# Lymphatus/caesium-clt

Measured on NVIDIA H100. Metric: megapixels/sec JPEG q=80 4K re-encode, higher is better.
Workload: dtype i32

## Files before the change

caesium-clt_b200/csrc/jpeg_gpuenc.cu:

```cuda
#include <cuda_runtime.h>
#include <cub/device/device_scan.cuh>
#include <cuda_pipeline.h>
#include <algorithm>
#include <chrono>
#include <cstring>
#include "jpeg_gpuenc.h"
#include "stream_wait.h"
#include "launch_timer.h"

namespace b200 {

using namespace ge;

__global__ void k_ge_groups(const Scan *__restrict__ scans, const uint32_t *__restrict__ meta, const int *__restrict__ evkey,
                            const int *__restrict__ prev, const uint32_t *__restrict__ tsum, uint32_t *__restrict__ gcount, uint32_t *__restrict__ hist)
{
    __shared__ uint32_t eob[16];
    const Scan s = scans[blockIdx.y];
    if (s.mode != MODE_AC_FIRST && s.mode != MODE_AC_REFINE) return;
    if ((int)(blockIdx.x * blockDim.x) > s.nblocks) return;
    if (threadIdx.x < 16) eob[threadIdx.x] = 0;
    __syncthreads();
    const int b = blockIdx.x * blockDim.x + threadIdx.x;
    if (b <= s.nblocks && (b == s.nblocks || meta_event(meta[s.unit_base + b]))) {
        int pg;
        if (b < s.nblocks) pg = prev[s.unit_base + b];
        else { const long long last = s.unit_base + s.nblocks - 1; pg = max(prev[last], evkey[last]); }
        const int pl = pg >= s.unit_base ? (int)(pg - s.unit_base) : -1;
        assign_groups(meta + s.unit_base, tsum + s.unit_base, s.nblocks, pl, b, gcount + s.unit_base,
                      [&](uint32_t c) { atomicAdd(&eob[eob_symbol(c) >> 4], 1u); });
    }
    __syncthreads();
    if (threadIdx.x < 16 && eob[threadIdx.x]) atomicAdd(&hist[((size_t)s.tab_base + 2 + s.tbl[0]) * 256 + (threadIdx.x << 4)], eob[threadIdx.x]);
}

__global__ void k_ge_tables(const uint32_t *__restrict__ hist, Table *__restrict__ tabs, DhtOut *__restrict__ dht, unsigned long long *__restrict__ tbits)
{
    __shared__ long long freq[257];
    __shared__ int codesize[257], others[257];
    __shared__ uint8_t bits[33];
    const int t = blockIdx.x, lane = threadIdx.x;
    const uint32_t *f = hist + (size_t)t * 256;
    for (int i = lane; i < 257; i += 32) { freq[i] = i < 256 ? (long long)f[i] : 1; codesize[i] = 0; others[i] = -1; }
    if (lane == 0) for (int i = 0; i < 33; i++) bits[i] = 0;
    __syncwarp();
    auto warp_argmin = [&](int exclude) {
        unsigned long long v = 1000000000ULL; int c = -1;
        for (int i = lane; i < 257; i += 32) { const unsigned long long fi = (unsigned long long)freq[i]; if (fi && fi <= v && i != exclude) { v = fi; c = i; } }
        const unsigned hi = (unsigned)(v >> 32), lo = (unsigned)v;
        const unsigned mhi = __reduce_min_sync(0xFFFFFFFFu, hi);
        const unsigned mlo = __reduce_min_sync(0xFFFFFFFFu, hi == mhi ? lo : 0xFFFFFFFFu);
        return __reduce_max_sync(0xFFFFFFFFu, (hi == mhi && lo == mlo) ? c : -1);
    };
    for (;;) {
        const int c1 = warp_argmin(-1);
        const int c2 = c1 < 0 ? -1 : warp_argmin(c1);
        if (c2 < 0) break;
        if (lane == 0) {
            int a = c1, b = c2;
            freq[a] += freq[b]; freq[b] = 0;
            codesize[a]++; while (others[a] >= 0) { a = others[a]; codesize[a]++; }
            others[a] = b;
            codesize[b]++; while (others[b] >= 0) { b = others[b]; codesize[b]++; }
        }
        __syncwarp();
    }
    if (lane == 0) {
        Table &T = tabs[t];
        for (int i = 0; i <= 256; i++) if (codesize[i]) bits[codesize[i] > 32 ? 32 : codesize[i]]++;
        for (int i = 32; i > 16; i--) while (bits[i] > 0) {
            int j = i - 2; while (bits[j] == 0) j--;
            bits[i] -= 2; bits[i - 1]++; bits[j + 1] += 2; bits[j]--;
        }
        int i = 16; while (i > 0 && bits[i] == 0) i--;
        if (i > 0) bits[i]--;
        int start[34];
        for (int l = 0; l < 34; l++) start[l] = 0;
        for (int s = 0; s <= 255; s++) if (codesize[s]) start[min(codesize[s], 32) + 1]++;
        for (int l = 1; l < 34; l++) start[l] += start[l - 1];
        const int p = start[33];
        for (int s = 0; s <= 255; s++) if (codesize[s]) T.vals[start[min(codesize[s], 32)]++] = (uint8_t)s;
        T.nvals = p;
        for (int k = 0; k < 17; k++) T.bits[k] = bits[k];
        for (int s = 0; s < 256; s++) T.code_len[s] = 0;
        uint32_t code = 0; int k = 0;
        for (int l = 1; l <= 16; l++) { for (int n = 0; n < bits[l]; n++, k++) T.code_len[T.vals[k]] = (code++ << 8) | (uint32_t)l; code <<= 1; }
        DhtOut &D = dht[t];
        D.nvals = p;
        for (int k2 = 0; k2 < 17; k2++) D.bits[k2] = bits[k2];
        for (int k2 = 0; k2 < p; k2++) D.vals[k2] = T.vals[k2];
    }
    __syncwarp();
    const int kind = (t & 3) >> 1;
    unsigned long long nb = 0;
    for (int i = lane; i < 256; i += 32) if (f[i]) nb += (unsigned long long)f[i] * ((tabs[t].code_len[i] & 0xFFu) + (unsigned)sym_extra_bits(kind, i));
    for (int d = 16; d; d >>= 1) nb += __shfl_xor_sync(0xFFFFFFFFu, nb, d);
    if (lane == 0) tbits[t] = nb;
}

__global__ void k_ge_scanout(const Scan *__restrict__ scans, int nscans, const unsigned long long *__restrict__ tbits, const uint32_t *__restrict__ corr,
                             uint32_t *__restrict__ total, ScanOut *__restrict__ so, uint32_t words_cap, uint32_t groups_cap, uint32_t *__restrict__ flags)
{
    const int lane = threadIdx.x;
    uint32_t wbase = 0, gbase = 0, abase = 0;
    for (int c0 = 0; c0 < nscans; c0 += 32) {
        const int i = c0 + lane;
        uint32_t tb = 0, na = 0;
        if (i < nscans) {
            tb = (uint32_t)(tbits[4 * i] + tbits[4 * i + 1] + tbits[4 * i + 2] + tbits[4 * i + 3] + corr[i]);
            na = scans[i].nruns ? (tb + 31) / 32 + scans[i].nruns : 0;
        }
        const uint32_t nbytes = (tb + 7) / 8, ng = (nbytes + 15) / 16, nw = i < nscans ? (tb + 31) / 32 + 1 : 0;
        uint32_t wi = nw, gi = i < nscans ? ng : 0, ai = na;
        for (int d = 1; d < 32; d <<= 1) {
            const uint32_t a = __shfl_up_sync(0xFFFFFFFFu, wi, d), b = __shfl_up_sync(0xFFFFFFFFu, gi, d), c = __shfl_up_sync(0xFFFFFFFFu, ai, d);
            if (lane >= d) { wi += a; gi += b; ai += c; }
        }
        if (i < nscans) {
            total[i] = tb;
            ScanOut o; o.total_bits = tb; o.nbytes = nbytes; o.ngroups = ng; o.group_base = gbase + gi - ng; o.word_base = wbase + wi - nw; o.arena_base = abase + ai - na;
            so[i] = o;
        }
        wbase += __shfl_sync(0xFFFFFFFFu, wi, 31); gbase += __shfl_sync(0xFFFFFFFFu, gi, 31); abase += __shfl_sync(0xFFFFFFFFu, ai, 31);
    }
    __syncwarp();
    const bool ovf = wbase > words_cap || gbase > groups_cap;
    if (lane == 0) { flags[0] = ovf ? 1u : 0u; flags[1] = wbase; flags[2] = gbase; flags[3] = 0; flags[4] = 0; }
    if (ovf) for (int i = lane; i < nscans; i += 32) { so[i].total_bits = 0; so[i].nbytes = 0; so[i].ngroups = 0; so[i].group_base = 0; so[i].word_base = 0; so[i].arena_base = 0; }
}

__global__ void k_ge_zero(const Scan *__restrict__ scans, const ScanOut *__restrict__ so, uint32_t *__restrict__ words, uint32_t *__restrict__ arena)
{
    const ScanOut o = so[blockIdx.y];
    if (!o.total_bits) return;
    const uint32_t n = (o.total_bits + 31) / 32 + 1, nruns = (uint32_t)scans[blockIdx.y].nruns, na = nruns ? n - 1 + nruns : 0;
    uint32_t *w = words + o.word_base, *a = arena + o.arena_base;
    for (uint32_t i = blockIdx.x * blockDim.x + threadIdx.x; i < max(n, na); i += gridDim.x * blockDim.x) {
        if (i < n) w[i] = 0;
        if (i < na) a[i] = 0;
    }
}

constexpr int TILE_PITCH = 72;
typedef int16_t Tile[ENC_THREADS][TILE_PITCH];

__device__ __forceinline__ void stage_tile(Tile &tile, const BlockComp &bc, int i0, int nblk)
{
    const uint4 *src = reinterpret_cast<const uint4 *>(bc.coef + bc.comp_off + (long long)i0 * 64);
    const int n = min(ENC_THREADS, nblk - i0) * 8;
#pragma unroll
    for (int k = 0; k < 8; k++) { const int q = threadIdx.x + k * ENC_THREADS; if (q < n) __pipeline_memcpy_async(&tile[q >> 3][(q & 7) * 8], src + q, 16); }
    __pipeline_commit();
}
__device__ __forceinline__ void wait_tile()
{
    __pipeline_wait_prior(0);
    __syncthreads();
}

__device__ __forceinline__ void stage_visits(EncVisit *vis, const BlockComp &bc)
{
    if ((int)threadIdx.x < bc.nscan) vis[threadIdx.x] = bc.visit[threadIdx.x];
}
__device__ __forceinline__ BlockRef ref_of(const EncVisit &v, const BlockComp &bc, const Tile &tile, int i0, int row, int col)
{
    BlockRef r;
    r.blk = tile[threadIdx.x]; r.prev = nullptr; r.slot = 0;
    if (v.mode == MODE_SEQ || v.mode == MODE_DC_FIRST) {
        const int p = enc_dc_prev(bc, v.ns, row, col);
        if (p >= i0 && p < i0 + ENC_THREADS) r.prev = tile[p - i0];
        else if (p >= 0) r.prev = bc.coef + bc.comp_off + (long long)p * 64;
    }
    return r;
}

template <class T>
__device__ __forceinline__ KindTabs<T> kind_tabs(T *tab, const EncVisit &v) { return KindTabs<T>{tab + ENC_DC_ENTRY, tab + v.ac_entry}; }

__device__ __forceinline__ Masks3 load_masks(const Masks3 *__restrict__ masks, const BlockComp &bc, int i)
{
    const unsigned long long *q = reinterpret_cast<const unsigned long long *>(masks + bc.mask_base + i);
    Masks3 M;
    M.m[0] = __ldg(q); M.m[1] = __ldg(q + 1); M.m[2] = __ldg(q + 2);
    return M;
}

struct SmemHist {
    KindTabs<uint32_t> h;
    __device__ void sym(int kind, int, int symbol, int, unsigned) { atomicAdd((kind ? h.ac : h.dc) + symbol, 1u); }
    __device__ void raw64(int, unsigned long long) {}
};
__global__ void __launch_bounds__(ENC_THREADS) k_geb_classify(const BlockComp *__restrict__ comps, uint32_t *__restrict__ meta, int *__restrict__ evkey,
                                                              uint32_t *__restrict__ tail, Masks3 *__restrict__ masks, uint32_t *__restrict__ hist, uint32_t *__restrict__ corr)
{
    __shared__ __align__(16) Tile tile;
    __shared__ uint32_t h[ENC_TAB_ENTRIES];
    __shared__ EncVisit vis[ENC_MAX_VISITS];
    __shared__ uint32_t vcorr[ENC_MAX_VISITS];
    const BlockComp &bc = comps[blockIdx.y];
    const int nblk = bc.bw * bc.bh, i0 = blockIdx.x * ENC_THREADS, i = i0 + threadIdx.x;
    if (i0 >= nblk) return;
    stage_tile(tile, bc, i0, nblk);
    for (int k = threadIdx.x; k < ENC_TAB_ENTRIES; k += ENC_THREADS) h[k] = 0;
    if (threadIdx.x < ENC_MAX_VISITS) vcorr[threadIdx.x] = 0;
    stage_visits(vis, bc);
    wait_tile();
    if (i < nblk) {
        const int row = i / bc.bw, col = i - row * bc.bw;
        const Masks3 M = make_masks3(tile[threadIdx.x]);
        masks[bc.mask_base + i] = M;
        for (int j = 0; j < bc.nscan; j++) {
            const EncVisit &v = vis[j];
            const int u = enc_unit_of(bc, v.ns, row, col);
            if (u < 0) continue;
            const uint32_t m = classify_m(v, M);
            const int g = v.unit_base + u;
            meta[g] = m; evkey[g] = meta_event(m) ? g : -1; tail[g] = (uint32_t)meta_tail(m);
            SmemHist sk{kind_tabs(h, v)};
            gen_block_m(v, v.tbl, ref_of(v, bc, tile, i0, row, col), M, 0, sk);
            const int nc = corr_bits_m(v, M);
            if (nc) atomicAdd(&vcorr[j], (uint32_t)nc);
        }
    }
    __syncthreads();
    if ((int)threadIdx.x < bc.nscan && vcorr[threadIdx.x]) atomicAdd(&corr[vis[threadIdx.x].scan], vcorr[threadIdx.x]);
    for (int k = threadIdx.x; k < ENC_TAB_ENTRIES; k += ENC_THREADS) {
        int symbol; const int t = enc_entry_table(bc, k, symbol);
        if (h[k]) atomicAdd(&hist[(size_t)t * 256 + symbol], h[k]);
    }
}

__global__ void __launch_bounds__(ENC_THREADS) k_geb_len(const BlockComp *__restrict__ comps, const uint32_t *__restrict__ gcount, const Table *__restrict__ tabs,
                                                         uint32_t *__restrict__ bitlen, const Masks3 *__restrict__ masks)
{
    __shared__ __align__(16) Tile tile;
    __shared__ uint8_t tl[ENC_TAB_ENTRIES];
    __shared__ EncVisit vis[ENC_MAX_VISITS];
    const BlockComp &bc = comps[blockIdx.y];
    const int nblk = bc.bw * bc.bh, i0 = blockIdx.x * ENC_THREADS, i = i0 + threadIdx.x;
    if (i0 >= nblk) return;
    stage_tile(tile, bc, i0, nblk);
    const Masks3 M = load_masks(masks, bc, min(i, nblk - 1));
    stage_visits(vis, bc);
    for (int k = threadIdx.x; k < ENC_TAB_ENTRIES; k += ENC_THREADS) {
        int symbol; const int t = enc_entry_table(bc, k, symbol);
        if (t >= 0) tl[k] = (uint8_t)tabs[t].code_len[symbol];
    }
    wait_tile();
    if (i >= nblk) return;
    const int row = i / bc.bw, col = i - row * bc.bw;
    for (int j = 0; j < bc.nscan; j++) {
        const EncVisit &v = vis[j];
        if (v.ns == 1) continue;
        const int u = enc_unit_of(bc, v.ns, row, col);
        if (u < 0) continue;
        LenSinkT<KindTabs<const uint8_t>> sk{kind_tabs<const uint8_t>(tl, v)};
        gen_block_m(v, v.tbl, ref_of(v, bc, tile, i0, row, col), M, gcount[v.unit_base + u], sk);
        bitlen[v.lu_base + u] = (uint32_t)sk.bits;
    }
}
constexpr int LEN_DC_THREADS = 256;
__global__ void __launch_bounds__(LEN_DC_THREADS) k_geb_len_dc(const BlockComp *__restrict__ comps, const Table *__restrict__ tabs, uint32_t *__restrict__ bitlen)
{
    const BlockComp &bc = comps[blockIdx.y];
    const int nblk = bc.bw * bc.bh, i = blockIdx.x * LEN_DC_THREADS + threadIdx.x;
    if (i >= nblk) return;
    const int row = i / bc.bw, col = i - row * bc.bw;
    const int16_t *cb = bc.coef + bc.comp_off;
    const Masks3 none{};
    for (int j = 0; j < bc.nscan; j++) {
        const EncVisit v = bc.visit[j];
        if (v.ns == 1) continue;
        const int p = enc_dc_prev(bc, v.ns, row, col);
        const BlockRef r{cb + (long long)i * 64, p >= 0 ? cb + (long long)p * 64 : nullptr, 0};
        LenSinkT<KindTabs<const uint32_t>> sk{KindTabs<const uint32_t>{tabs[bc.tab[ENC_AC_SLOTS]].code_len, nullptr}};
        gen_block_m(v, v.tbl, r, none, 0, sk);
        bitlen[v.lu_base + enc_unit_of(bc, v.ns, row, col)] = (uint32_t)sk.bits;
    }
}

__device__ __forceinline__ uint32_t cta_exclusive_sum(uint32_t x, uint32_t *wsum , uint32_t &total)
{
    const int lane = threadIdx.x & 31, w = threadIdx.x >> 5;
    uint32_t inc = x;
    for (int d = 1; d < 32; d <<= 1) { const uint32_t y = __shfl_up_sync(0xFFFFFFFFu, inc, d); if (lane >= d) inc += y; }
    if (lane == 31) wsum[w] = inc;
    __syncthreads();
    uint32_t base = 0, tot = 0;
#pragma unroll
    for (int k = 0; k < ENC_THREADS / 32; k++) { const uint32_t sk = wsum[k]; if (k < w) base += sk; tot += sk; }
    total = tot;
    return base + inc - x;
}

constexpr int ENC_SLOT_WORDS = 8;
__global__ void __launch_bounds__(ENC_THREADS) k_geb_emit(const BlockComp *__restrict__ comps, const uint32_t *__restrict__ gcount, const Table *__restrict__ tabs,
                                                          const uint32_t *__restrict__ bitoff, uint32_t *__restrict__ words, const Masks3 *__restrict__ masks, const ScanOut *__restrict__ so,
                                                          const uint32_t *__restrict__ flags, uint32_t *__restrict__ arena, uint32_t *__restrict__ cursor,
                                                          uint32_t *__restrict__ runlen, uint32_t *__restrict__ runpos)
{
    __shared__ __align__(16) Tile tile;
    __shared__ uint32_t tc[ENC_TAB_ENTRIES];
    __shared__ EncVisit vis[ENC_MAX_VISITS];
    __shared__ uint32_t vword[ENC_MAX_VISITS], vbit0[ENC_MAX_VISITS];
    __shared__ uint32_t slot[ENC_SLOT_WORDS][ENC_THREADS];
    __shared__ uint32_t wsum[ENC_THREADS / 32], run_word;
    if (flags[0]) return;
    const BlockComp &bc = comps[blockIdx.y];
    const int nblk = bc.bw * bc.bh, i0 = blockIdx.x * ENC_THREADS, i = i0 + threadIdx.x;
    if (i0 >= nblk) return;
    const bool live = i < nblk;
    stage_tile(tile, bc, i0, nblk);
    const Masks3 M = load_masks(masks, bc, min(i, nblk - 1));
    stage_visits(vis, bc);
    if ((int)threadIdx.x < bc.nscan) {
        const EncVisit &v = bc.visit[threadIdx.x];
        const ScanOut &o = so[v.scan];
        vword[threadIdx.x] = v.ns > 1 ? o.word_base : o.arena_base; vbit0[threadIdx.x] = v.ns > 1 ? bitoff[v.lu_base] : 0;
    }
    for (int k = threadIdx.x; k < ENC_TAB_ENTRIES; k += ENC_THREADS) {
        int symbol; const int t = enc_entry_table(bc, k, symbol);
        if (t >= 0) tc[k] = tabs[t].code_len[symbol];
    }
    wait_tile();
    const int row = i / bc.bw, col = i - row * bc.bw;
    auto orw = [&](long long w, uint32_t v) { if (v) atomicOr(&words[w], v); };
    auto stw = [&](long long w, uint32_t v) { words[w] = v; };
    auto ora = [&](long long w, uint32_t v) { if (v) atomicOr(&arena[w], v); };
    auto sta = [&](long long w, uint32_t v) { arena[w] = v; };
    auto sls = [&](long long w, uint32_t v) { if (w < ENC_SLOT_WORDS) slot[w][threadIdx.x] = v; };
    typedef KindTabs<const uint32_t> KT;
    for (int j = 0; j < bc.nscan; j++) {
        const EncVisit &v = vis[j];
        const int u = live ? enc_unit_of(bc, v.ns, row, col) : -1;
        if (v.ns > 1) {
            if (u < 0) continue;
            EmitSink<decltype(orw), decltype(stw), KT> sk(kind_tabs<const uint32_t>(tc, v), orw, stw, (long long)vword[j], (unsigned long long)(bitoff[v.lu_base + u] - vbit0[j]));
            gen_block_m(v, v.tbl, ref_of(v, bc, tile, i0, row, col), M, gcount[v.unit_base + u], sk);
            sk.finish();
            continue;
        }
        uint32_t nb = 0;
        if (u >= 0) {
            EmitSink<decltype(sls), decltype(sls), KT> sk(kind_tabs<const uint32_t>(tc, v), sls, sls, 0, 0);
            gen_block_m(v, v.tbl, ref_of(v, bc, tile, i0, row, col), M, gcount[v.unit_base + u], sk);
            sk.finish();
            nb = (uint32_t)sk.bits_written(0);
        }
        uint32_t L;
        const uint32_t off = cta_exclusive_sum(nb, wsum, L);
        if (threadIdx.x == 0) {
            const uint32_t a = vword[j] + atomicAdd(&cursor[v.scan], (L + 31) / 32);
            run_word = a; runlen[v.run_base + blockIdx.x] = L; runpos[v.run_base + blockIdx.x] = a;
        }
        __syncthreads();
        const unsigned long long at = (unsigned long long)run_word * 32 + off;
        if (nb <= ENC_SLOT_WORDS * 32) place_bits([&](long long k) { return slot[k][threadIdx.x]; }, nb, at, ora, sta);
        else {
            EmitSink<decltype(ora), decltype(sta), KT> sk(kind_tabs<const uint32_t>(tc, v), ora, sta, 0, at);
            gen_block_m(v, v.tbl, ref_of(v, bc, tile, i0, row, col), M, gcount[v.unit_base + u], sk);
            sk.finish();
        }
    }
}

constexpr int PLACE_THREADS = 128;
__global__ void __launch_bounds__(PLACE_THREADS) k_ge_place(const Scan *__restrict__ scans, const ScanOut *__restrict__ so, const uint32_t *__restrict__ runlen,
                                                            const uint32_t *__restrict__ runoff, const uint32_t *__restrict__ runpos, const uint32_t *__restrict__ arena,
                                                            uint32_t *__restrict__ words, const uint32_t *__restrict__ flags)
{
    if (flags[0]) return;
    const int nruns = scans[blockIdx.y].nruns, x = blockIdx.x * (PLACE_THREADS / 32) + (threadIdx.x >> 5);
    if (x >= nruns) return;
    const int r0 = scans[blockIdx.y].run_base, r = r0 + x;
    const uint32_t *src = arena + runpos[r];
    uint32_t *dst = words + so[blockIdx.y].word_base;
    place_bits([&](long long k) { return src[k]; }, runlen[r], runoff[r] - runoff[r0],
               [&](long long w, uint32_t v) { atomicOr(&dst[w], v); }, [&](long long w, uint32_t v) { dst[w] = v; }, threadIdx.x & 31, 32);
}

__device__ __forceinline__ uint32_t scan_byte(const uint32_t *__restrict__ w, uint32_t i, uint32_t nbytes, uint32_t total_bits)
{
    uint32_t b = (w[i >> 2] >> (24 - 8 * (i & 3))) & 0xFF;
    if (i == nbytes - 1 && (total_bits & 7)) b |= (1u << (8 - (total_bits & 7))) - 1u;
    return b;
}

__global__ void k_ge_ffcount(const ScanOut *__restrict__ so, int nscans, const uint32_t *__restrict__ words, uint32_t *__restrict__ ffcount, uint32_t groups_cap,
                             const uint32_t *__restrict__ flags)
{
    if ((int)blockIdx.y == nscans) {
        const uint32_t used = flags[0] ? 0u : flags[2];
        for (uint32_t g = used + blockIdx.x * blockDim.x + threadIdx.x; g < groups_cap; g += gridDim.x * blockDim.x) ffcount[g] = 0;
        return;
    }
    const ScanOut o = so[blockIdx.y];
    const uint32_t *w = words + o.word_base;
    for (uint32_t g = blockIdx.x * blockDim.x + threadIdx.x; g < o.ngroups; g += gridDim.x * blockDim.x) {
        uint32_t n = 0;
        for (uint32_t i = g * 16; i < g * 16 + 16 && i < o.nbytes; i++) n += scan_byte(w, i, o.nbytes, o.total_bits) == 0xFF;
        ffcount[o.group_base + g] = n;
    }
}

__global__ void k_ge_layout(const ScanOut *__restrict__ so, int scans_per_image, int nimages, const uint32_t *__restrict__ ffcount, const uint32_t *__restrict__ ffoff,
                            uint32_t *__restrict__ out_off, uint32_t *__restrict__ out_len, uint32_t out_image_stride, uint32_t *__restrict__ flags)
{
    const int im = blockIdx.x * blockDim.x + threadIdx.x;
    if (im >= nimages) return;
    uint32_t off = 0;
    for (int k = 0; k < scans_per_image; k++) {
        const int si = im * scans_per_image + k;
        const ScanOut o = so[si];
        uint32_t ff = 0;
        if (o.ngroups) { const uint32_t lastg = o.group_base + o.ngroups - 1; ff = ffoff[lastg] + ffcount[lastg] - ffoff[o.group_base]; }
        out_off[si] = off; out_len[si] = o.nbytes + ff;
        off += o.nbytes + ff;
    }
    atomicMax(&flags[3], off);
    if (off > out_image_stride) atomicOr(&flags[4], 1u);
}

__global__ void k_ge_scatter(const ScanOut *__restrict__ so, const uint32_t *__restrict__ words, const uint32_t *__restrict__ ffoff,
                             const uint32_t *__restrict__ out_off, uint8_t *__restrict__ out, int scans_per_image, size_t out_image_stride, const uint32_t *__restrict__ flags)
{
    if (flags[4]) return;
    const ScanOut o = so[blockIdx.y];
    const uint32_t *w = words + o.word_base;
    uint8_t *base = out + (size_t)(blockIdx.y / scans_per_image) * out_image_stride + out_off[blockIdx.y];
    for (uint32_t g = blockIdx.x * blockDim.x + threadIdx.x; g < o.ngroups; g += gridDim.x * blockDim.x) {
        uint8_t *dst = base + (size_t)g * 16 + (ffoff[o.group_base + g] - ffoff[o.group_base]);
        for (uint32_t i = g * 16; i < g * 16 + 16 && i < o.nbytes; i++) {
            const uint32_t b = scan_byte(w, i, o.nbytes, o.total_bits);
            *dst++ = (uint8_t)b;
            if (b == 0xFF) *dst++ = 0;
        }
    }
}

__global__ void k_ge_fill_dummy(int16_t *__restrict__ coef, long long comp_off, int bw, int bh, int rbw, int rbh, int hs)
{
    const int i = blockIdx.x * blockDim.x + threadIdx.x;
    if (i >= bw * bh) return;
    const int row = i / bw, col = i - row * bw;
    if (row < rbh && col < rbw) return;
    int r = row, c = col;
    while (r >= rbh || c >= rbw) { if (r >= rbh) { c = (c / hs) * hs + hs - 1; r--; } else c = rbw - 1; }
    int16_t *base = coef + comp_off;
    int16_t *dst = base + ((long long)row * bw + col) * 64;
    const int16_t dc = base[((long long)r * bw + c) * 64];
    for (int k = 1; k < 64; k++) dst[k] = 0;
    dst[0] = dc;
}

static inline size_t align_up(size_t v, size_t a) { return (v + a - 1) / a * a; }
static inline int cdiv(long long a, long long b) { return (int)((a + b - 1) / b); }

GpuEncoder::~GpuEncoder()
{
    if (ev_sizes) cudaEventDestroy((cudaEvent_t)ev_sizes);
}

bool GpuEncoder::size_back_buffers(size_t image_bytes, std::string &err)
{
    const int NS = (int)plan.scans.size();
    auto grow = [&](auto &buf, size_t need) { return buf.reserve(need, Grow::Pow2Half, err, &generation); };
    auto grow_arena = [&]() { return grow(d_arena, ((size_t)words_cap + (size_t)plan.total_runs) * 4 + 64); };
    if (nimg != cap_nimg) { cap_nimg = nimg; est_image_bytes = 0; }
    if (image_bytes <= est_image_bytes && words_cap) return grow_arena();
    est_image_bytes = image_bytes + image_bytes / 8;
    image_bytes = est_image_bytes;
    words_cap = (uint32_t)std::min<size_t>((size_t)nimg * (image_bytes / 4 + 1) + 2 * (size_t)NS + 64, 0xFFFFFF00u);
    groups_cap = (uint32_t)((size_t)words_cap / 4 + NS + 1);
    out_stride = align_up(image_bytes + image_bytes / 8 + 1024, 256);
    if (!grow_arena() || !grow(d_words, (size_t)words_cap * 4 + 64) || !grow(d_ffcount, (size_t)groups_cap * 4 + 4) || !grow(d_ffoff, (size_t)groups_cap * 4 + 4) ||
        !grow(d_out, out_stride * nimg)) return false;
    size_t tb3 = 0; cub::DeviceScan::ExclusiveSum((void *)nullptr, tb3, d_ffcount.get(), d_ffoff.get(), (int)groups_cap, (cudaStream_t)0);
    return grow(d_temp, tb3 + 256);
}

bool GpuEncoder::prepare(const JpegGeom &g, bool progressive, int16_t *const *d_coefs, int nimages, void *stream_, size_t out_bytes_hint, std::string &err)
{
    cudaStream_t st = (cudaStream_t)stream_;
    geom = g; prog = progressive;
    std::vector<const int16_t *> bases(d_coefs, d_coefs + nimages);
    coef_bases.assign(d_coefs, d_coefs + nimages);
    gpuenc_plan(g, progressive, bases.data(), nimages, plan);
    nimg = nimages;
    const int NS = (int)plan.scans.size();
    const long long U = plan.total_units, LU = std::max(plan.total_lunits, 1ll);
    const int R = std::max(plan.total_runs, 1);
    if (U >= (1ll << 31)) { err = "batch too large for the entropy encoder"; return false; }
    overflow = false;
    for (auto &sc_ : plan.scans) if (!masks_cover(sc_.mode, sc_.Al)) { err = "scan script outside the device encoder's mask range"; overflow = true; return false; }
    if (!plan.on_chip) { err = "scan script outside the device encoder's on-chip table slots"; overflow = true; return false; }
    if (!ev_sizes) { cudaEvent_t e; CU(cudaEventCreateWithFlags(&e, cudaEventDisableTiming | (stream_wait_mode() == 0 ? 0 : cudaEventBlockingSync))); ev_sizes = e; }
    auto grow = [&](auto &buf, size_t need) { return buf.reserve(need, Grow::Pow2Half, err, &generation); };
    const int NC = (int)plan.comps.size();
    if (!grow(d_scans, NS * sizeof(Scan)) || !grow(d_comps, NC * sizeof(BlockComp)) ||
        !grow(d_meta, U * 4) || !grow(d_evkey, U * 4) || !grow(d_prev, U * 4) || !grow(d_tail, U * 4) || !grow(d_tsum, U * 4) ||
        !grow(d_gcount, U * 4) || !grow(d_bitlen, LU * 4) || !grow(d_bitoff, LU * 4) || !grow(d_corr, (size_t)NS * 4) || !grow(d_tbits, (size_t)NS * 4 * 8) ||
        !grow(d_cursor, (size_t)NS * 4) || !grow(d_runlen, (size_t)R * 4) || !grow(d_runoff, (size_t)R * 4) || !grow(d_runpos, (size_t)R * 4) ||
        !grow(d_hist, (size_t)NS * 4 * 256 * 4) || !grow(d_tabs, (size_t)NS * 4 * sizeof(Table)) || !grow(d_dht, (size_t)NS * 4 * sizeof(DhtOut)) ||
        !grow(d_total, (size_t)NS * 4) || !grow(d_so, (size_t)NS * sizeof(ScanOut)) || !grow(d_outoff, (size_t)NS * 4) || !grow(d_outlen, (size_t)NS * 4) ||
        !grow(d_flags, 64) || !grow(d_masks, (size_t)plan.total_comp_blocks * sizeof(Masks3))) return false;
    o_scans = 0; o_total = o_scans + align_up((size_t)NS * sizeof(Scan), 256); o_outlen = o_total + align_up((size_t)NS * 4, 256);
    o_dht = o_outlen + align_up((size_t)NS * 4, 256); o_comps = o_dht + align_up((size_t)NS * 4 * sizeof(DhtOut), 256);
    o_flags = o_comps + align_up((size_t)NC * sizeof(BlockComp), 256);
    const size_t small_bytes = o_flags + 256;
    if (!grow(h_small, small_bytes)) return false;
    size_t tb1 = 0, tb2 = 0, tb3 = 0, tb4 = 0;
    cub::DeviceScan::ExclusiveScan((void *)nullptr, tb1, d_evkey.get(), d_prev.get(), cub::Max(), -1, (int)U, st);
    cub::DeviceScan::ExclusiveSum((void *)nullptr, tb2, d_tail.get(), d_tsum.get(), (int)U, st);
    cub::DeviceScan::ExclusiveSum((void *)nullptr, tb3, d_bitlen.get(), d_bitoff.get(), (int)LU, st);
    cub::DeviceScan::ExclusiveSum((void *)nullptr, tb4, d_runlen.get(), d_runoff.get(), R, st);
    if (!grow(d_temp, std::max(std::max(tb1, tb2), std::max(tb3, tb4)) + 256)) return false;
    const size_t coef_bytes = (size_t)g.total_coefs * 2;
    if (coef_bytes != learned_for) { learned_for = coef_bytes; learned_image_bytes = 0; }
    size_t est = out_bytes_hint ? out_bytes_hint / nimages + out_bytes_hint / nimages / 4 : coef_bytes / 3;
    est = std::max(est, learned_image_bytes + learned_image_bytes / 8) + 8192;
    est = std::min(est, coef_bytes * 2 + (size_t)plan.scans_per_image * 64 + 8192);
    if (!size_back_buffers(est, err)) return false;
    memcpy(h_small + o_scans, plan.scans.data(), NS * sizeof(Scan));
    memcpy(h_small + o_comps, plan.comps.data(), NC * sizeof(BlockComp));
    (void)st;
    return true;
}

bool GpuEncoder::upload(void *stream_, std::string &err)
{
    cudaStream_t st = (cudaStream_t)stream_;
    const int NS = (int)plan.scans.size(), NC = (int)plan.comps.size();
    CU(cudaMemcpyAsync(d_scans, h_small + o_scans, NS * sizeof(Scan), cudaMemcpyHostToDevice, st));
    CU(cudaMemcpyAsync(d_comps, h_small + o_comps, NC * sizeof(BlockComp), cudaMemcpyHostToDevice, st));
    return true;
}

unsigned long long GpuEncoder::signature() const
{
    unsigned long long h = 1469598103934665603ull;
    auto mix = [&](unsigned long long v) { h = (h ^ v) * 1099511628211ull; };
    mix((unsigned long long)nimg); mix((unsigned long long)plan.scans.size()); mix((unsigned long long)plan.comps.size()); mix((unsigned long long)plan.total_units);
    mix((unsigned long long)plan.max_comp_blocks); mix((unsigned long long)plan.scans_per_image); mix(words_cap); mix(groups_cap); mix(out_stride); mix(generation);
    mix((unsigned long long)geom.width); mix((unsigned long long)geom.height); mix(prog ? 1 : 0);
    for (int c = 0; c < geom.ncomp; c++) { mix((unsigned long long)geom.bw[c]); mix((unsigned long long)geom.bh[c]); mix((unsigned long long)geom.rbw[c]); mix((unsigned long long)geom.rbh[c]); mix((unsigned long long)geom.hs[c]); }
    for (auto pb : coef_bases) mix((unsigned long long)(uintptr_t)pb);
    int max_units = 0; for (auto &sc : plan.scans) max_units = std::max(max_units, sc.nblocks);
    mix((unsigned long long)max_units);
    mix((unsigned long long)plan.total_lunits); mix((unsigned long long)plan.total_runs); mix((unsigned long long)plan.max_runs);
    return h;
}

bool GpuEncoder::enqueue_sizes(void *stream_, std::string &err)
{
    cudaStream_t st = (cudaStream_t)stream_;
    const int NS = (int)plan.scans.size();
    uint32_t *h_total = reinterpret_cast<uint32_t *>(h_small + o_total), *h_flags = reinterpret_cast<uint32_t *>(h_small + o_flags);
    k_ge_scanout<<<1, 32, 0, st>>>(d_scans, NS, d_tbits, d_corr, d_total, d_so, words_cap, groups_cap, d_flags);
    LT_MARK("k_ge_scanout");
    CU(cudaMemcpyAsync(h_total, d_total, (size_t)NS * 4, cudaMemcpyDeviceToHost, st));
    CU(cudaMemcpyAsync(h_flags, d_flags, 12, cudaMemcpyDeviceToHost, st));
    LT_MARK("copy");
    return true;
}
bool GpuEncoder::mark_sizes(void *stream_, std::string &err)
{
    CU(cudaEventRecord((cudaEvent_t)ev_sizes, (cudaStream_t)stream_));
    return true;
}

bool GpuEncoder::enqueue_back(void *stream_, std::string &err)
{
    cudaStream_t st = (cudaStream_t)stream_;
    const int NS = (int)plan.scans.size(), NC = (int)plan.comps.size();
    uint32_t *h_flags = reinterpret_cast<uint32_t *>(h_small + o_flags);
    const dim3 gb(cdiv(plan.max_comp_blocks, ENC_THREADS), NC);
    int n = 6;
    if (plan.total_lunits) {
        bool dc_only = true;
        for (auto &sc : plan.scans) if (sc.ns > 1 && sc.mode != MODE_DC_FIRST) dc_only = false;
        if (dc_only) {
            k_geb_len_dc<<<dim3(cdiv(plan.max_comp_blocks, LEN_DC_THREADS), NC), LEN_DC_THREADS, 0, st>>>(d_comps, d_tabs, d_bitlen);
            LT_MARK("k_geb_len_dc");
        } else {
            k_geb_len<<<gb, ENC_THREADS, 0, st>>>(d_comps, d_gcount, d_tabs, d_bitlen, d_masks);
            LT_MARK("k_geb_len");
        }
        size_t tb = d_temp.capacity();
        cub::DeviceScan::ExclusiveSum(d_temp, tb, d_bitlen.get(), d_bitoff.get(), (int)plan.total_lunits, st);
        LT_MARK("cub_scan");
        n += 2;
    }
    CU(cudaMemsetAsync(d_cursor, 0, (size_t)NS * 4, st));
    LT_MARK("memset");
    k_ge_zero<<<dim3(64, NS), 256, 0, st>>>(d_scans, d_so, d_words, d_arena);
    LT_MARK("k_ge_zero");
    k_geb_emit<<<gb, ENC_THREADS, 0, st>>>(d_comps, d_gcount, d_tabs, d_bitoff, d_words, d_masks, d_so, d_flags, d_arena, d_cursor, d_runlen, d_runpos);
    LT_MARK("k_geb_emit");
    if (plan.total_runs) {
        size_t tb = d_temp.capacity();
        cub::DeviceScan::ExclusiveSum(d_temp, tb, d_runlen.get(), d_runoff.get(), plan.total_runs, st);
        LT_MARK("cub_scan");
        k_ge_place<<<dim3(cdiv(plan.max_runs, PLACE_THREADS / 32), NS), PLACE_THREADS, 0, st>>>(d_scans, d_so, d_runlen, d_runoff, d_runpos, d_arena, d_words, d_flags);
        LT_MARK("k_ge_place");
        n += 2;
    }
    k_ge_ffcount<<<dim3(32, NS + 1), 128, 0, st>>>(d_so, NS, d_words, d_ffcount, groups_cap, d_flags);
    LT_MARK("k_ge_ffcount");
    size_t tb = d_temp.capacity();
    cub::DeviceScan::ExclusiveSum(d_temp, tb, d_ffcount.get(), d_ffoff.get(), (int)groups_cap, st);
    LT_MARK("cub_scan");
    k_ge_layout<<<cdiv(nimg, 64), 64, 0, st>>>(d_so, plan.scans_per_image, nimg, d_ffcount, d_ffoff, d_outoff, d_outlen, (uint32_t)out_stride, d_flags);
    LT_MARK("k_ge_layout");
    k_ge_scatter<<<dim3(32, NS), 128, 0, st>>>(d_so, d_words, d_ffoff, d_outoff, d_out, plan.scans_per_image, out_stride, d_flags);
    LT_MARK("k_ge_scatter");
    CU(cudaMemcpyAsync(h_small + o_outlen, d_outlen, (size_t)NS * 4, cudaMemcpyDeviceToHost, st));
    CU(cudaMemcpyAsync(h_small + o_dht, d_dht, (size_t)NS * 4 * sizeof(DhtOut), cudaMemcpyDeviceToHost, st));
    CU(cudaMemcpyAsync(h_flags + 4, d_flags, 32, cudaMemcpyDeviceToHost, st));
    CU(cudaGetLastError());
    launches += n;
    return true;
}

bool GpuEncoder::enqueue(void *stream_, bool fill_dummy, std::string &err)
{
    return enqueue_front(stream_, fill_dummy, err) && enqueue_sizes(stream_, err) && mark_sizes(stream_, err) && enqueue_back(stream_, err);
}

bool GpuEncoder::enqueue_front(void *stream_, bool fill_dummy, std::string &err)
{
    cudaStream_t st = (cudaStream_t)stream_;
    const JpegGeom &g = geom;
    const int NS = (int)plan.scans.size(), NC = (int)plan.comps.size();
    const long long U = plan.total_units;
    int max_units = 0; for (auto &s : plan.scans) max_units = std::max(max_units, s.nblocks);
    launches = 0;
    const dim3 gb(cdiv(plan.max_comp_blocks, ENC_THREADS), NC);
    if (fill_dummy) {
        for (int im = 0; im < nimg; im++) for (int cc = 0; cc < g.ncomp; cc++) {
            if (g.rbw[cc] == g.bw[cc] && g.rbh[cc] == g.bh[cc]) continue;
            k_ge_fill_dummy<<<cdiv((long long)g.bw[cc] * g.bh[cc], 256), 256, 0, st>>>(coef_bases[im], g.comp_offset[cc], g.bw[cc], g.bh[cc], g.rbw[cc], g.rbh[cc], g.hs[cc]);
            LT_MARK("k_ge_fill_dummy");
            launches++;
        }
    }
    const dim3 gu1(cdiv(max_units + 1, 128), NS);
    CU(cudaMemsetAsync(d_hist, 0, (size_t)NS * 4 * 256 * 4, st));
    LT_MARK("memset");
    CU(cudaMemsetAsync(d_corr, 0, (size_t)NS * 4, st));
    LT_MARK("memset");
    k_geb_classify<<<gb, ENC_THREADS, 0, st>>>(d_comps, d_meta, d_evkey, d_tail, d_masks, d_hist, d_corr);
    LT_MARK("k_geb_classify");
    size_t tb = d_temp.capacity();
    cub::DeviceScan::ExclusiveScan(d_temp, tb, d_evkey.get(), d_prev.get(), cub::Max(), -1, (int)U, st);
    LT_MARK("cub_scan");
    tb = d_temp.capacity();
    cub::DeviceScan::ExclusiveSum(d_temp, tb, d_tail.get(), d_tsum.get(), (int)U, st);
    LT_MARK("cub_scan");
    CU(cudaMemsetAsync(d_gcount, 0, U * 4, st));
    LT_MARK("memset");
    k_ge_groups<<<gu1, 128, 0, st>>>(d_scans, d_meta, d_evkey, d_prev, d_tsum, d_gcount, d_hist);
    LT_MARK("k_ge_groups");
    k_ge_tables<<<NS * 4, 32, 0, st>>>(d_hist, d_tabs, d_dht, d_tbits);
    LT_MARK("k_ge_tables");
    launches += 5;
    CU(cudaGetLastError());
    return true;
}

bool GpuEncoder::finish(void *stream_, bool fetch, std::string &err)
{
    cudaStream_t st = (cudaStream_t)stream_;
    const int NS = (int)plan.scans.size(), spi = plan.scans_per_image;
    uint32_t *h_total = reinterpret_cast<uint32_t *>(h_small + o_total), *h_flags = reinterpret_cast<uint32_t *>(h_small + o_flags);
    uint32_t *h_outlen = reinterpret_cast<uint32_t *>(h_small + o_outlen);
    const DhtOut *h_dht = reinterpret_cast<const DhtOut *>(h_small + o_dht);
    for (int attempt = 0;; attempt++) {
        const auto tw0 = std::chrono::steady_clock::now();
        if (fetch) { CU(event_wait((cudaEvent_t)ev_sizes)); } else { CU(stream_wait(st)); }
        wait_sizes_ms = std::chrono::duration<double, std::milli>(std::chrono::steady_clock::now() - tw0).count();
        size_t img_max = 0, img = 0;
        for (int si = 0; si < NS; si++) { img += (h_total[si] + 7) / 8; if ((si + 1) % spi == 0) { img_max = std::max(img_max, img); img = 0; } }
        if (h_flags[0]) {
            if (attempt >= 3) { err = "entropy encoder could not size its buffers"; return false; }
            CU(stream_wait(st));
            if (!size_back_buffers(img_max + img_max / 16 + 4096, err)) return false;
            retries++;
            if (!enqueue_sizes(st, err) || !mark_sizes(st, err) || !enqueue_back(st, err)) return false;
            continue;
        }
        if (fetch) {
            copy_bytes = std::min(out_stride, align_up(img_max + img_max / 8 + 256, 256));
            if (!h_out.reserve(copy_bytes * nimg, Grow::Pow2Half, err, &generation)) return false;
            for (int im = 0; im < nimg; im++) CU(cudaMemcpyAsync(h_out + (size_t)im * copy_bytes, d_out + (size_t)im * out_stride, copy_bytes, cudaMemcpyDeviceToHost, st));
            CU(cudaGetLastError());
            const auto tw1 = std::chrono::steady_clock::now();
            CU(stream_wait(st));
            wait_final_ms = std::chrono::duration<double, std::milli>(std::chrono::steady_clock::now() - tw1).count();
        }
        if (h_flags[4 + 4]) {
            if (attempt >= 3) { err = "entropy encoder could not size its output"; return false; }
            if (!size_back_buffers((size_t)h_flags[4 + 3] + 4096, err)) return false;
            retries++;
            if (!enqueue_sizes(st, err) || !mark_sizes(st, err) || !enqueue_back(st, err)) return false;
            continue;
        }
        learned_image_bytes = std::max<size_t>(learned_image_bytes, h_flags[4 + 3]);
        if (fetch) {
            bool shortc = false;
            for (int im = 0; im < nimg && !shortc; im++) { size_t tot = 0; for (int k = 0; k < spi; k++) tot += h_outlen[im * spi + k]; shortc = tot > copy_bytes; }
            if (shortc) {
                if (!h_out.reserve(out_stride * nimg, Grow::Pow2Half, err, &generation)) return false;
                copy_bytes = out_stride;
                for (int j = 0; j < nimg; j++) CU(cudaMemcpyAsync(h_out + (size_t)j * copy_bytes, d_out + (size_t)j * out_stride, copy_bytes, cudaMemcpyDeviceToHost, st));
                CU(stream_wait(st));
            }
        }
        break;
    }
    results.assign((size_t)NS, EncodedScan());
    for (int si = 0; si < NS; si++) {
        EncodedScan &e = results[si];
        const int im = si / spi, k = si % spi;
        e.def = plan.defs[k];
        size_t off = 0; for (int j = 0; j < k; j++) off += h_outlen[im * spi + j];
        e.data = fetch ? h_out + (size_t)im * copy_bytes + off : nullptr; e.len = h_outlen[si];
        bool need[2][2]; jpeg_scan_tables_needed(geom, prog, e.def, need);
        for (int kind = 0; kind < 2; kind++) for (int t = 0; t < 2; t++) {
            e.has_tab[kind][t] = need[kind][t];
            const DhtOut &D = h_dht[(size_t)si * 4 + kind * 2 + t];
            memcpy(e.bits[kind][t], D.bits, 17); memcpy(e.vals[kind][t], D.vals, 256); e.nvals[kind][t] = D.nvals;
        }
    }
    return true;
}

bool GpuEncoder::encode(const JpegGeom &g, bool progressive, int16_t *const *d_coefs, int nimages, void *stream_, bool fill_dummy, std::string &err, size_t out_bytes_hint)
{
    return prepare(g, progressive, d_coefs, nimages, stream_, out_bytes_hint, err) && upload(stream_, err) && enqueue(stream_, fill_dummy, err) && finish(stream_, true, err);
}

}
```

caesium-clt_b200/csrc/jpeg_gpuenc_core.h:

```cpp
#pragma once
#include <cstdint>

#if defined(__CUDACC__)
#define GE_HD __host__ __device__ __forceinline__
#else
#define GE_HD inline
#endif

namespace b200 {
namespace ge {

enum ScanMode { MODE_SEQ = 0, MODE_DC_FIRST = 1, MODE_AC_FIRST = 2, MODE_AC_REFINE = 3 };

constexpr int EOBRUN_MAX = 0x7FFF;
constexpr int CORR_FLUSH = 1000 - 64 + 1;

struct Scan {
    const int16_t *coef;
    int mode, ns, Ss, Se, Al;
    int comp[3];
    int hs[3], vs[3], bw[3];
    long long comp_off[3];
    int tbl[3];
    int mcux, mcuy, blocks_per_mcu;
// ... 232 lines not shown
        if ((mB >> k) & 1ull) { pend64 = (pend64 << 1) | (unsigned)(t & 1); npend++; continue; }
        sk.sym(1, tbl, (r << 4) + 1, 1, neg ? 0u : 1u);
        if (npend) { sk.raw64(npend, pend64); npend = 0; pend64 = 0; }
        r = 0;
    }
    if (group_count) gen_eob_token(group_count, tbl, sk);
    if (npend) sk.raw64(npend, pend64);
}
template <class Sink>
GE_HD void gen_block(const Scan &s, const BlockRef &b, unsigned group_count, Sink &sk)
{
    if (s.mode == MODE_DC_FIRST) { Masks3 none; none.m[0] = none.m[1] = none.m[2] = 0; gen_block_m(s, s.tbl[b.slot], b, none, group_count, sk); return; }
    gen_block_m(s, s.tbl[b.slot], b, make_masks3(b.blk), group_count, sk);
}

struct ScanTabs {
    const Table *t = nullptr;
    ScanTabs() = default;
    GE_HD ScanTabs(const Table *p) : t(p) {}
    GE_HD uint32_t operator()(int kind, int tbl, int symbol) const { return t[kind * 2 + tbl].code_len[symbol]; }
};
template <class T>
struct KindTabs {
    T *dc, *ac;
    GE_HD uint32_t operator()(int kind, int, int symbol) const { return (kind ? ac : dc)[symbol]; }
};

template <class AddFn>
struct HistSink {
    AddFn add;
    GE_HD explicit HistSink(AddFn f) : add(f) {}
    GE_HD void sym(int kind, int tbl, int symbol, int, unsigned) { add((kind * 2 + tbl) * 256 + symbol); }
    GE_HD void raw64(int, unsigned long long) {}
};

template <class Tabs = ScanTabs>
struct LenSinkT {
    Tabs tabs;
    unsigned long long bits = 0;
    GE_HD void sym(int kind, int tbl, int symbol, int nb, unsigned) { bits += (tabs(kind, tbl, symbol) & 0xFFu) + nb; }
    GE_HD void raw64(int nb, unsigned long long) { bits += nb; }
};
using LenSink = LenSinkT<>;

GE_HD uint32_t shl_or_zero(uint32_t v, int s)
{
#if defined(__CUDA_ARCH__)
    return __funnelshift_lc(0u, v, (unsigned)s);
#else
    return s >= 32 ? 0u : v << s;
#endif
}

template <class OrFn, class StFn = OrFn, class Tabs = ScanTabs>
struct EmitSink {
    Tabs tabs;
    OrFn orw;
    StFn stw;
    long long wpos, first;
    uint32_t cur = 0; int n;
    GE_HD EmitSink(Tabs t, OrFn f, StFn g, long long word_base, unsigned long long bitoff)
        : tabs(t), orw(f), stw(g), wpos(word_base + (long long)(bitoff >> 5)), first(wpos), n((int)(bitoff & 31)) {}
    GE_HD EmitSink(Tabs t, OrFn f, long long word_base, unsigned long long bitoff) : EmitSink(t, f, f, word_base, bitoff) {}
    GE_HD void put(uint32_t code, int len)
    {
        if (!len) return;
        const int fill = n + len;
        if (fill < 32) { cur |= code << (32 - fill); n = fill; return; }
        const int r = fill - 32;
        const uint32_t w = cur | (code >> r);
        if (wpos == first) orw(wpos, w); else stw(wpos, w);
        wpos++;
        cur = shl_or_zero(code, 32 - r); n = r;
    }
    GE_HD void sym(int kind, int tbl, int symbol, int nb, unsigned extra)
    {
        const uint32_t e = tabs(kind, tbl, symbol);
        put(((e >> 8) << nb) | (extra & ((1u << nb) - 1u)), (int)(e & 0xFFu) + nb);
    }
    GE_HD void raw64(int nb, unsigned long long v)
    {
        if (nb > 32) { put((unsigned)(v >> 32), nb - 32); put((unsigned)v, 32); } else put((unsigned)v, nb);
    }
    GE_HD void finish() { if (n > 0) orw(wpos, cur); }
    GE_HD unsigned long long bits_written(long long word_base) const { return (unsigned long long)(wpos - word_base) * 32 + n; }
};

template <class Src, class OrFn, class StFn>
GE_HD void place_bits(Src src, unsigned long long nbits, unsigned long long bitoff, OrFn &&orw, StFn &&stw, int k0 = 0, int dk = 1)
{
    if (!nbits) return;
    const int s = (int)(bitoff & 31);
    const long long w0 = (long long)(bitoff >> 5), nsrc = (long long)((nbits + 31) / 32), nout = (long long)((s + nbits + 31) / 32);
    for (long long k = k0; k < nout; k += dk) {
        const uint32_t hi = k > 0 ? src(k - 1) : 0u, lo = k < nsrc ? src(k) : 0u;
        const uint32_t v = s ? (hi << (32 - s)) | (lo >> s) : lo;
        if (k == 0 || k == nout - 1) { if (v) orw(w0 + k, v); }
        else stw(w0 + k, v);
    }
}

struct NoCount { GE_HD void operator()(uint32_t) const {} };
template <class CountFn = NoCount>
GE_HD void assign_groups(const uint32_t *meta, const uint32_t *tsum, int nblocks, int prev_ev, int b, uint32_t *gcount, CountFn &&counted = CountFn())
{
    auto group = [&](int j, uint32_t c) { gcount[j] = c; counted(c); };
    int gs = prev_ev < 0 ? 0 : (meta_contrib(meta[prev_ev]) ? prev_ev : prev_ev + 1);
    if (gs >= b) return;
    const int count = b - gs;
    const uint32_t tend = b < nblocks ? tsum[b] : tsum[nblocks - 1] + (uint32_t)meta_tail(meta[nblocks - 1]);
    const uint32_t tailbits = tend - tsum[gs];
    if (count < EOBRUN_MAX && tailbits <= (uint32_t)CORR_FLUSH) { group(gs, (uint32_t)count); return; }
    int start = gs, n = 0; unsigned be = 0;
    for (int j = gs; j < b; j++) {
        n++; be += (unsigned)meta_tail(meta[j]);
        if (n == EOBRUN_MAX || be > (unsigned)CORR_FLUSH) { group(start, (uint32_t)n); start = j + 1; n = 0; be = 0; }
    }
    if (n > 0) group(start, (uint32_t)n);
}

GE_HD void build_table(const uint32_t *freq_in, Table &t, int *codesize , int *others , long long *freq )
{
    uint8_t bits[33];
    for (int i = 0; i < 33; i++) bits[i] = 0;
    for (int i = 0; i < 256; i++) { freq[i] = freq_in[i]; codesize[i] = 0; others[i] = -1; }
    freq[256] = 1; codesize[256] = 0; others[256] = -1;
    for (;;) {
        int c1 = -1, c2 = -1; long long v = 1000000000LL;
        for (int i = 0; i <= 256; i++) if (freq[i] && freq[i] <= v) { v = freq[i]; c1 = i; }
        v = 1000000000LL;
        for (int i = 0; i <= 256; i++) if (freq[i] && freq[i] <= v && i != c1) { v = freq[i]; c2 = i; }
        if (c2 < 0) break;
        freq[c1] += freq[c2]; freq[c2] = 0;
        codesize[c1]++; while (others[c1] >= 0) { c1 = others[c1]; codesize[c1]++; }
        others[c1] = c2;
        codesize[c2]++; while (others[c2] >= 0) { c2 = others[c2]; codesize[c2]++; }
    }
    for (int i = 0; i <= 256; i++) if (codesize[i]) bits[codesize[i] > 32 ? 32 : codesize[i]]++;
    for (int i = 32; i > 16; i--) while (bits[i] > 0) {
        int j = i - 2; while (bits[j] == 0) j--;
        bits[i] -= 2; bits[i - 1]++; bits[j + 1] += 2; bits[j]--;
    }
    int i = 16; while (i > 0 && bits[i] == 0) i--;
    if (i > 0) bits[i]--;
    for (int k = 0; k < 17; k++) t.bits[k] = bits[k];
    int p = 0;
    for (int l = 1; l <= 32; l++) for (int s = 0; s <= 255; s++) if (codesize[s] == l) t.vals[p++] = (uint8_t)s;
    t.nvals = p;
    for (int s = 0; s < 256; s++) t.code_len[s] = 0;
    uint32_t code = 0; int k = 0;
    for (int l = 1; l <= 16; l++) { for (int n = 0; n < t.bits[l]; n++, k++) t.code_len[t.vals[k]] = (code++ << 8) | (uint32_t)l; code <<= 1; }
}

}
}
```

Baseline: 45880.

## Vectorize byte-stuffing count and scatter via uint4 loads and shared-memory staging

The 0xFF counting and byte-stuffing scatter kernels now load each 16-byte group as a single uint4, byte-swap it, and count 0xFF bytes with SIMD byte compares instead of looping byte by byte. The scatter kernel writes stuffed bytes into a shared-memory staging buffer, then flushes the block's contiguous output range with aligned 32-bit stores. This replaces scattered per-byte global writes with coalesced word writes. Per-scan word buffers are padded to 16-byte multiples so the vector loads stay in bounds, which slightly enlarges the words allocation and adds block-wide syncs.

After: 46990, median of 6. +2.4%, better.

```diff
diff --git a/caesium-clt_b200/csrc/jpeg_gpuenc.cu b/caesium-clt_b200/csrc/jpeg_gpuenc.cu
--- a/caesium-clt_b200/csrc/jpeg_gpuenc.cu
+++ b/caesium-clt_b200/csrc/jpeg_gpuenc.cu
@@ -110,7 +110,7 @@
             tb = (uint32_t)(tbits[4 * i] + tbits[4 * i + 1] + tbits[4 * i + 2] + tbits[4 * i + 3] + corr[i]);
             na = scans[i].nruns ? (tb + 31) / 32 + scans[i].nruns : 0;
         }
-        const uint32_t nbytes = (tb + 7) / 8, ng = (nbytes + 15) / 16, nw = i < nscans ? (tb + 31) / 32 + 1 : 0;
+        const uint32_t nbytes = (tb + 7) / 8, ng = (nbytes + 15) / 16, nw = i < nscans ? scan_buffer_words(tb) : 0;
         uint32_t wi = nw, gi = i < nscans ? ng : 0, ai = na;
         for (int d = 1; d < 32; d <<= 1) {
             const uint32_t a = __shfl_up_sync(0xFFFFFFFFu, wi, d), b = __shfl_up_sync(0xFFFFFFFFu, gi, d), c = __shfl_up_sync(0xFFFFFFFFu, ai, d);
@@ -379,15 +379,11 @@
                [&](long long w, uint32_t v) { atomicOr(&dst[w], v); }, [&](long long w, uint32_t v) { dst[w] = v; }, threadIdx.x & 31, 32);
 }
 
-__device__ __forceinline__ uint32_t scan_byte(const uint32_t *__restrict__ w, uint32_t i, uint32_t nbytes, uint32_t total_bits)
-{
-    uint32_t b = (w[i >> 2] >> (24 - 8 * (i & 3))) & 0xFF;
-    if (i == nbytes - 1 && (total_bits & 7)) b |= (1u << (8 - (total_bits & 7))) - 1u;
-    return b;
-}
-
-__global__ void k_ge_ffcount(const ScanOut *__restrict__ so, int nscans, const uint32_t *__restrict__ words, uint32_t *__restrict__ ffcount, uint32_t groups_cap,
-                             const uint32_t *__restrict__ flags)
+constexpr int STUFF_THREADS = 128, STUFF_X = 32;
+__device__ __forceinline__ ScanGroup load_scan_group(const uint32_t *w, uint32_t g) { const uint4 q = reinterpret_cast<const uint4 *>(w)[g]; return ScanGroup{{q.x, q.y, q.z, q.w}}; }
+
+__global__ void __launch_bounds__(STUFF_THREADS) k_ge_ffcount(const ScanOut *__restrict__ so, int nscans, const uint32_t *__restrict__ words, uint32_t *__restrict__ ffcount,
+                                                              uint32_t groups_cap, const uint32_t *__restrict__ flags)
 {
     if ((int)blockIdx.y == nscans) {
         const uint32_t used = flags[0] ? 0u : flags[2];
@@ -396,11 +392,8 @@
     }
     const ScanOut o = so[blockIdx.y];
     const uint32_t *w = words + o.word_base;
-    for (uint32_t g = blockIdx.x * blockDim.x + threadIdx.x; g < o.ngroups; g += gridDim.x * blockDim.x) {
-        uint32_t n = 0;
-        for (uint32_t i = g * 16; i < g * 16 + 16 && i < o.nbytes; i++) n += scan_byte(w, i, o.nbytes, o.total_bits) == 0xFF;
-        ffcount[o.group_base + g] = n;
-    }
+    for (uint32_t g = blockIdx.x * blockDim.x + threadIdx.x; g < o.ngroups; g += gridDim.x * blockDim.x)
+        ffcount[o.group_base + g] = stuff_count_group(load_scan_group(w, g), g, o.nbytes, o.total_bits);
 }
 
 __global__ void k_ge_layout(const ScanOut *__restrict__ so, int scans_per_image, int nimages, const uint32_t *__restrict__ ffcount, const uint32_t *__restrict__ ffoff,
@@ -421,20 +414,27 @@
     if (off > out_image_stride) atomicOr(&flags[4], 1u);
 }
 
-__global__ void k_ge_scatter(const ScanOut *__restrict__ so, const uint32_t *__restrict__ words, const uint32_t *__restrict__ ffoff,
-                             const uint32_t *__restrict__ out_off, uint8_t *__restrict__ out, int scans_per_image, size_t out_image_stride, const uint32_t *__restrict__ flags)
-{
+__global__ void __launch_bounds__(STUFF_THREADS) k_ge_scatter(const ScanOut *__restrict__ so, const uint32_t *__restrict__ words, const uint32_t *__restrict__ ffoff,
+                                                              const uint32_t *__restrict__ out_off, uint8_t *__restrict__ out, int scans_per_image, size_t out_image_stride,
+                                                              const uint32_t *__restrict__ flags)
+{
+    __shared__ uint32_t sbuf[STUFF_THREADS * 8 + 1];
+    __shared__ uint32_t range_end;
     if (flags[4]) return;
     const ScanOut o = so[blockIdx.y];
-    const uint32_t *w = words + o.word_base;
-    uint8_t *base = out + (size_t)(blockIdx.y / scans_per_image) * out_image_stride + out_off[blockIdx.y];
-    for (uint32_t g = blockIdx.x * blockDim.x + threadIdx.x; g < o.ngroups; g += gridDim.x * blockDim.x) {
-        uint8_t *dst = base + (size_t)g * 16 + (ffoff[o.group_base + g] - ffoff[o.group_base]);
-        for (uint32_t i = g * 16; i < g * 16 + 16 && i < o.nbytes; i++) {
-            const uint32_t b = scan_byte(w, i, o.nbytes, o.total_bits);
-            *dst++ = (uint8_t)b;
-            if (b == 0xFF) *dst++ = 0;
-        }
+    const uint32_t *w = words + o.word_base, *off = ffoff + o.group_base;
+    const uint32_t start = out_off[blockIdx.y], base = off[0];
+    uint8_t *img = out + (size_t)(blockIdx.y / scans_per_image) * out_image_stride, *sb = reinterpret_cast<uint8_t *>(sbuf);
+    for (uint32_t g0 = blockIdx.x * STUFF_THREADS; g0 < o.ngroups; g0 += gridDim.x * STUFF_THREADS) {
+        const uint32_t g = g0 + threadIdx.x;
+        const uint32_t first = start + g0 * 16 + (off[g0] - base), aligned = first & ~3u;
+        if (g < o.ngroups) {
+            const uint32_t e = stuff_place_group(load_scan_group(w, g), g, o.nbytes, o.total_bits, start + g * 16 + (off[g] - base), aligned, sb);
+            if (g == g0 + STUFF_THREADS - 1 || g == o.ngroups - 1) range_end = e;
+        }
+        __syncthreads();
+        stuff_store(sbuf, aligned, first, range_end, threadIdx.x, STUFF_THREADS, img);
+        __syncthreads();
     }
 }
 
@@ -470,7 +470,7 @@
     if (image_bytes <= est_image_bytes && words_cap) return grow_arena();
     est_image_bytes = image_bytes + image_bytes / 8;
     image_bytes = est_image_bytes;
-    words_cap = (uint32_t)std::min<size_t>((size_t)nimg * (image_bytes / 4 + 1) + 2 * (size_t)NS + 64, 0xFFFFFF00u);
+    words_cap = (uint32_t)std::min<size_t>((size_t)nimg * (image_bytes / 4 + 1) + 5 * (size_t)NS + 64, 0xFFFFFF00u);
     groups_cap = (uint32_t)((size_t)words_cap / 4 + NS + 1);
     out_stride = align_up(image_bytes + image_bytes / 8 + 1024, 256);
     if (!grow_arena() || !grow(d_words, (size_t)words_cap * 4 + 64) || !grow(d_ffcount, (size_t)groups_cap * 4 + 4) || !grow(d_ffoff, (size_t)groups_cap * 4 + 4) ||
@@ -605,14 +605,14 @@
         LT_MARK("k_ge_place");
         n += 2;
     }
-    k_ge_ffcount<<<dim3(32, NS + 1), 128, 0, st>>>(d_so, NS, d_words, d_ffcount, groups_cap, d_flags);
+    k_ge_ffcount<<<dim3(STUFF_X, NS + 1), STUFF_THREADS, 0, st>>>(d_so, NS, d_words, d_ffcount, groups_cap, d_flags);
     LT_MARK("k_ge_ffcount");
     size_t tb = d_temp.capacity();
     cub::DeviceScan::ExclusiveSum(d_temp, tb, d_ffcount.get(), d_ffoff.get(), (int)groups_cap, st);
     LT_MARK("cub_scan");
     k_ge_layout<<<cdiv(nimg, 64), 64, 0, st>>>(d_so, plan.scans_per_image, nimg, d_ffcount, d_ffoff, d_outoff, d_outlen, (uint32_t)out_stride, d_flags);
     LT_MARK("k_ge_layout");
-    k_ge_scatter<<<dim3(32, NS), 128, 0, st>>>(d_so, d_words, d_ffoff, d_outoff, d_out, plan.scans_per_image, out_stride, d_flags);
+    k_ge_scatter<<<dim3(STUFF_X, NS), STUFF_THREADS, 0, st>>>(d_so, d_words, d_ffoff, d_outoff, d_out, plan.scans_per_image, out_stride, d_flags);
     LT_MARK("k_ge_scatter");
     CU(cudaMemcpyAsync(h_small + o_outlen, d_outlen, (size_t)NS * 4, cudaMemcpyDeviceToHost, st));
     CU(cudaMemcpyAsync(h_small + o_dht, d_dht, (size_t)NS * 4 * sizeof(DhtOut), cudaMemcpyDeviceToHost, st));
diff --git a/caesium-clt_b200/csrc/jpeg_gpuenc_core.h b/caesium-clt_b200/csrc/jpeg_gpuenc_core.h
--- a/caesium-clt_b200/csrc/jpeg_gpuenc_core.h
+++ b/caesium-clt_b200/csrc/jpeg_gpuenc_core.h
@@ -408,5 +408,73 @@
     for (int l = 1; l <= 16; l++) { for (int n = 0; n < t.bits[l]; n++, k++) t.code_len[t.vals[k]] = (code++ << 8) | (uint32_t)l; code <<= 1; }
 }
 
-}
-}
+struct ScanGroup { uint32_t w[4]; };
+
+GE_HD uint32_t scan_buffer_words(uint32_t total_bits) { return ((total_bits + 31) / 32 + 4) & ~3u; }
+
+GE_HD uint32_t bswap32(uint32_t x)
+{
+#if defined(__CUDA_ARCH__)
+    return __byte_perm(x, 0u, 0x0123);
+#else
+    return __builtin_bswap32(x);
+#endif
+}
+GE_HD uint32_t ff_bytes(uint32_t x)
+{
+#if defined(__CUDA_ARCH__)
+    return (uint32_t)__popc(__vcmpeq4(x, 0xFFFFFFFFu)) >> 3;
+#else
+    uint32_t c = 0;
+    for (int t = 0; t < 4; t++) c += ((x >> (8 * t)) & 0xFFu) == 0xFFu;
+    return c;
+#endif
+}
+
+GE_HD uint32_t stream_group(ScanGroup &q, uint32_t g, uint32_t nbytes, uint32_t total_bits)
+{
+    const uint32_t n = nbytes - 16 * g < 16 ? nbytes - 16 * g : 16;
+    for (int k = 0; k < 4; k++) {
+        const uint32_t keep = n > 4u * k ? n - 4u * k : 0u;
+        q.w[k] = bswap32(q.w[k]) & (keep >= 4 ? 0xFFFFFFFFu : (1u << (8 * keep)) - 1u);
+    }
+    if (16 * g + n == nbytes && (total_bits & 7)) {
+        const uint32_t pad = (1u << (8 - (total_bits & 7))) - 1u, t = n - 1;
+        for (int k = 0; k < 4; k++) if ((uint32_t)k == t >> 2) q.w[k] |= pad << (8 * (t & 3));
+    }
+    return n;
+}
+
+GE_HD uint32_t stuff_count_group(ScanGroup q, uint32_t g, uint32_t nbytes, uint32_t total_bits)
+{
+    stream_group(q, g, nbytes, total_bits);
+    return ff_bytes(q.w[0]) + ff_bytes(q.w[1]) + ff_bytes(q.w[2]) + ff_bytes(q.w[3]);
+}
+
+GE_HD uint32_t stuff_place_group(ScanGroup q, uint32_t g, uint32_t nbytes, uint32_t total_bits, uint32_t o, uint32_t aligned, uint8_t *sb)
+{
+    const uint32_t n = stream_group(q, g, nbytes, total_bits);
+#if defined(__CUDA_ARCH__)
+#pragma unroll
+#endif
+    for (int t = 0; t < 16; t++) {
+        const uint32_t b = (q.w[t >> 2] >> (8 * (t & 3))) & 0xFFu;
+        if ((uint32_t)t < n) {
+            sb[o++ - aligned] = (uint8_t)b;
+            if (b == 0xFFu) sb[o++ - aligned] = 0;
+        }
+    }
+    return o;
+}
+
+GE_HD void stuff_store(const uint32_t *sbuf, uint32_t aligned, uint32_t first, uint32_t end, uint32_t tid, uint32_t nthreads, uint8_t *out)
+{
+    for (uint32_t a = aligned + 4 * tid; a < end; a += 4 * nthreads) {
+        const uint32_t w = sbuf[(a - aligned) >> 2];
+        if (a >= first && a + 4 <= end) *reinterpret_cast<uint32_t *>(out + a) = w;
+        else for (uint32_t t = 0; t < 4; t++) if (a + t >= first && a + t < end) out[a + t] = (uint8_t)(w >> (8 * t));
+    }
+}
+
+}
+}
```
